# bcosm/MonteCarloOptionsPricer

Hardware: AMD Instinct MI355X
Metric: Mpaths/sec at 252 steps (higher is better)
Workload: dtype f64; 1 GPU; C2: European call, GBM, 10M paths x 252 steps per GPU, fp64 matrix written; collective=none, seed=20251031

## Files before the change

### include/mcgpu_debug.h

```cpp
#ifndef MCGPU_DEBUG_H
#define MCGPU_DEBUG_H
#include "mcgpu.h"
#ifdef __cplusplus
extern "C" {
#endif

int mcg_debug_eval(mcg_ctx* ctx, int fn, const double* x, double* y, int64_t n);
int mcg_debug_lsm_hooks(mcg_ctx* ctx, long long spin_limit, int poll_delay);
int mcg_debug_lsm_date_fault(mcg_ctx* ctx, int mode, int date, int workgroup, int delay, long long spin_limit);
int mcg_debug_batch_budget(mcg_ctx* ctx, size_t bytes);
int mcg_debug_coalesce_slots(int max_slots);
int mcg_debug_coalesce_selftest(int n_threads, int calls_per_thread, int* wrong);
int mcg_debug_peer_decision(int same_process, int bus_id_resolves, int same_device, int can_access_peer);
int mcg_debug_shm_attach(const char* name, int n_ranks, int rank, double timeout_s, void** handle);
int mcg_debug_shm_barrier(void* handle);
int mcg_debug_shm_poison(void* handle);
int mcg_debug_shm_detach(void* handle);

#ifdef __cplusplus
}
#endif
#endif
```

### montecarlooptionspricer_amd/_native.py

```python
from __future__ import annotations

import ctypes as C
import os
import sys

_HERE = os.path.dirname(os.path.abspath(__file__))
_LIB = os.environ.get("MCG_LIB") or os.path.join(_HERE, "lib", "libmcgpu.so")

MCG_OK = 0
K_GBM, K_RBERGOMI, K_PAYOFF, K_LSM_SWEEP, K_LSM_SOLVE, K_TRANSPOSE, K_ASYM, K_MARTINGALE, K_BRANCHING, K_BATCH, K_EXOTIC, K_HESTON, K_MULTI, K_LOCALVOL = range(14)
KERNEL_NAMES = {K_GBM: "gbm", K_RBERGOMI: "rbergomi", K_PAYOFF: "payoff", K_LSM_SWEEP: "lsm_sweep",
                K_LSM_SOLVE: "lsm_solve", K_TRANSPOSE: "transpose", K_ASYM: "asymptotic", K_MARTINGALE: "martingale", K_BRANCHING: "branching", K_BATCH: "batch_rows",
                K_EXOTIC: "exotic", K_HESTON: "heston", K_MULTI: "multi", K_LOCALVOL: "localvol"}
K_LSM_APPLY = 14

LSM_POLICY_STRIDE = 20
POL_CONTINUE, POL_EXERCISE_RULE, POL_TERMINAL = range(3)

(X_ASIAN_ARITH_FIXED, X_ASIAN_ARITH_FLOAT, X_ASIAN_GEO_FIXED, X_ASIAN_GEO_FLOAT, X_LOOKBACK_FIXED, X_LOOKBACK_FLOAT,
 X_BARRIER_UP_OUT, X_BARRIER_UP_IN, X_BARRIER_DOWN_OUT, X_BARRIER_DOWN_IN) = range(10)
EXOTIC_KINDS = {"asian_arith_fixed": X_ASIAN_ARITH_FIXED, "asian_arith_float": X_ASIAN_ARITH_FLOAT,
                "asian_geo_fixed": X_ASIAN_GEO_FIXED, "asian_geo_float": X_ASIAN_GEO_FLOAT,
                "lookback_fixed": X_LOOKBACK_FIXED, "lookback_float": X_LOOKBACK_FLOAT,
                "barrier_up_out": X_BARRIER_UP_OUT, "barrier_up_in": X_BARRIER_UP_IN,
# ... 100 lines not shown
                raise

    newer("mcg_comm_shm_peer_mailbox", [vp, C.c_int, C.POINTER(C.c_int)])
    newer("mcg_debug_shm_attach", [C.c_char_p, C.c_int, C.c_int, C.c_double, C.POINTER(vp)])
    newer("mcg_debug_shm_barrier", [vp])
    newer("mcg_debug_shm_poison", [vp])
    newer("mcg_debug_shm_detach", [vp])
    newer("mcg_lsm_one_launch_reset", [vp])
    newer("mcg_debug_lsm_hooks", [vp, C.c_longlong, C.c_int])
    newer("mcg_comm_info", [vp] + [C.POINTER(C.c_int)] * 4)
    newer("mcg_timing_select", [vp, C.c_uint])
    newer("mcg_stats", [C.POINTER(Stats), C.c_int])
    newer("mcg_debug_lsm_date_fault", [vp, C.c_int, C.c_int, C.c_int, C.c_int, C.c_longlong])
    newer("mcg_debug_batch_budget", [vp, C.c_size_t])
    newer("mcg_debug_peer_decision", [C.c_int] * 4)
    newer("mcg_probe_write_ceiling", [vp, C.c_int64, C.c_int, C.c_int, C.POINTER(C.c_double), C.POINTER(C.c_double)])
    newer("mcg_generator_clock_arm", [vp, C.c_int])
    newer("mcg_generator_clock", [vp, C.POINTER(C.c_double), C.POINTER(C.c_int), C.POINTER(C.c_double), C.POINTER(C.c_double)])
    newer("mcg_row_features", [C.POINTER(C.c_double), C.c_size_t, C.POINTER(C.c_double), C.POINTER(C.c_double)])
    newer("mcg_row_build", [C.POINTER(C.c_double), C.c_size_t, C.c_double, C.c_double, C.c_double, C.c_int, C.c_double,
                            C.POINTER(Row), C.POINTER(C.c_double)])
    newer("mcg_batch_price_rows6", [vp, C.POINTER(Row), C.POINTER(C.c_double), C.c_int64, C.c_int, C.c_double, C.c_double, C.c_int,
                                    C.c_int, C.c_int, C.c_uint64, C.POINTER(C.c_double)])
    L.mcg_paths_gbm.argtypes = [vp, C.c_uint64, C.c_double, C.c_double, C.c_double, C.c_double, C.c_int,
                                C.c_uint64, C.c_int64, C.POINTER(vp)]
    L.mcg_paths_gbm_payoff.argtypes = [vp, C.c_uint64, C.c_double, C.c_double, C.c_double, C.c_double, C.c_int,
                                       C.c_uint64, C.c_int64, C.c_double, C.c_int, C.POINTER(vp)]
    L.mcg_paths_rbergomi.argtypes = [vp, C.c_uint64] + [C.c_double] * 7 + [C.c_int, C.c_uint64, C.c_int64,
                                                                          C.POINTER(vp)]
    L.mcg_paths_rbergomi_payoff.argtypes = [vp, C.c_uint64] + [C.c_double] * 7 + [C.c_int, C.c_uint64, C.c_int64,
                                                                                 C.c_double, C.c_int, C.POINTER(vp)]
    L.mcg_paths_heston.argtypes = [vp, C.c_uint64] + [C.c_double] * 8 + [C.c_int, C.c_uint64, C.c_int64, C.POINTER(vp), C.POINTER(vp)]
    L.mcg_paths_heston_payoff.argtypes = [vp, C.c_uint64] + [C.c_double] * 8 + [C.c_int, C.c_uint64, C.c_int64, C.c_double, C.c_int,
                                          C.POINTER(vp), C.POINTER(vp)]
    L.mcg_paths_heston_qe.argtypes = L.mcg_paths_heston.argtypes
    L.mcg_paths_heston_qe_payoff.argtypes = L.mcg_paths_heston_payoff.argtypes
    L.mcg_paths_bates.argtypes = [vp, C.c_uint64] + [C.c_double] * 11 + [C.c_int, C.c_uint64, C.c_int64, C.c_int, C.POINTER(vp),
                                                                          C.POINTER(vp)]
    L.mcg_paths_bates_payoff.argtypes = [vp, C.c_uint64] + [C.c_double] * 11 + [C.c_int, C.c_uint64, C.c_int64, C.c_int, C.c_double,
                                                                                 C.c_int, C.POINTER(vp), C.POINTER(vp)]
    L.mcg_cholesky_corr.argtypes = [dp, C.c_int, dp]
    L.mcg_paths_gbm_multi.argtypes = [vp, C.c_uint64, C.c_int, dp, C.c_double, dp, dp, dp, C.c_double, C.c_int, C.c_uint64, C.c_int64,
                                      C.c_int, dp, C.POINTER(vp), C.POINTER(vp)]
    L.mcg_paths_combine.argtypes = [vp, C.POINTER(vp), C.c_int, C.c_int, dp, C.POINTER(vp)]
    lv = [vp, C.c_uint64, C.c_double, C.c_double, C.c_double, dp, C.c_int, C.c_double, C.c_double, C.c_int, dp, C.c_double, C.c_int,
          C.c_uint64, C.c_int64]
# ... 56 lines not shown
```

### montecarlooptionspricer_amd/csrc/fastmath.hpp

```cpp
#pragma once
#include <hip/hip_runtime.h>
#include <stdint.h>

#include "philox.hpp"

namespace mcg {
namespace fm {

constexpr int LOG_TAB_ENTRIES = 1024;
constexpr int SINCOS_BITS = 10;
constexpr int SINCOS_TAB_ENTRIES = 1 << SINCOS_BITS;
constexpr int EXP2_TAB_ENTRIES = 256;
constexpr int TABLE_UNITS = LOG_TAB_ENTRIES + SINCOS_TAB_ENTRIES + EXP2_TAB_ENTRIES / 2;

struct Tables {
    static constexpr int SC_BITS = SINCOS_BITS;
    double2 log[LOG_TAB_ENTRIES];
    double2 sincos[SINCOS_TAB_ENTRIES];
    double exp2[EXP2_TAB_ENTRIES];
};
template <int BITS>
struct NormalTables {
    static_assert(BITS >= 6 && BITS <= SINCOS_BITS, "a sub-sampling of the 1024-entry table");
    static constexpr int SC_BITS = BITS;
// ... 252 lines not shown
    z1 = rad * s;
}

template <class T>
__device__ __forceinline__ void box_muller_pair_affine(uint32_t wa, uint32_t wb, const T* tab, double scale,
                                                       double shift, double& a0, double& a1) {
    const double rad = scale * sqrt_pos(neg2log(radius_u01(wa, wb), tab->log));
    double c, s;
    sincos_table<T::SC_BITS>(wb, tab->sincos, c, s);
    a0 = __builtin_fma(rad, c, shift);
    a1 = __builtin_fma(rad, s, shift);
}

template <class T>
__device__ __forceinline__ void box_muller_pair_affine_scaled(uint32_t wa, uint32_t wb, const T* tab, const LogScale& L,
                                                              double shift, double& a0, double& a1) {
    const double rad = sqrt_pos(neg2log_scaled(radius_u01(wa, wb), tab->log, L));
    double c, s;
    sincos_table<T::SC_BITS>(wb, tab->sincos, c, s);
    a0 = __builtin_fma(rad, c, shift);
    a1 = __builtin_fma(rad, s, shift);
}

template <bool EAGER = false>
__device__ __forceinline__ void normal_quad_words(const Philox4 w, const Tables* tab, double (&z)[4], double amp0, double amp1);

template <bool EAGER = false>
__device__ __forceinline__ void normal_quad_fast(uint32_t k0, uint32_t k1, uint64_t path, uint32_t block,
                                                 uint32_t stream, const Tables* tab, double (&z)[4], double amp0 = 1.0,
                                                 double amp1 = 1.0) {
    normal_quad_words<EAGER>(philox4x32_10((uint32_t)path, (uint32_t)(path >> 32), block, stream, k0, k1), tab, z, amp0, amp1);
}
template <bool EAGER = false>
__device__ __forceinline__ void normal_quad_fast(uint32_t k0, uint32_t k1, const PhiloxLane& L, uint32_t block, const Tables* tab,
                                                 double (&z)[4], double amp0 = 1.0, double amp1 = 1.0) {
    normal_quad_words<EAGER>(philox4x32_10_path(L, block, k0, k1), tab, z, amp0, amp1);
}

template <bool EAGER>
__device__ __forceinline__ void normal_quad_words(const Philox4 w, const Tables* tab, double (&z)[4], double amp0, double amp1) {
    if constexpr (!EAGER) {
        box_muller_pair_affine(w.w0, w.w1, tab, amp0, 0.0, z[0], z[1]);
        box_muller_pair_affine(w.w2, w.w3, tab, amp1, 0.0, z[2], z[3]);
        return;
    }
    const LogSplit s0 = log_split(radius_u01(w.w0, w.w1)), s1 = log_split(radius_u01(w.w2, w.w3));
// ... 41 lines not shown
```

### montecarlooptionspricer_amd/csrc/kernels_debug.hip

```cpp
#include "devmath.hpp"
#include "fastmath.hpp"
#include "mcg_internal.hpp"

namespace mcg {

__global__ __launch_bounds__(256) void k_debug_eval(int fn, const double* x, double* y, int64_t n,
                                                    const double2* gtab) {
    __shared__ fm::Tables tabs;
    const fm::Tables* tab = &tabs;
    fm::load_tables(&tabs, gtab);
    __syncthreads();
    const int64_t i = (int64_t)blockIdx.x * 256 + threadIdx.x;
    if (i >= n) return;
    const double v = x[i];
    double a = 0.0, b = 0.0;
    double z[4] = {0.0, 0.0, 0.0, 0.0};
    switch (fn) {
        case 0: a = fm::scaled_exp(1.0, v); break;
        case 1: a = fm::neg2log(v, tab->log); break;
        case 2: a = fm::sqrt_pos(v); break;
        case 3: fm::sincos_table((uint32_t)v, tab->sincos, a, b); break;
        case 4: fm::normal_quad_fast(1u, 0u, (uint64_t)v, 0u, STREAM_PRICE, tab, z); break;
        case 6: a = fm::scaled_exp_small(1.0, v); break;
        case 7: a = fm::scaled_exp_small6(1.0, v); break;
        case 8: fm::exp2_pair(v, v + 96.0, tab, a, b); break;
        case 9: fm::normal_quad_fast<true>(1u, 0u, (uint64_t)v, 0u, STREAM_PRICE, tab, z); break;
        default: normal_quad_ref(1u, 0u, (uint64_t)v, 0u, STREAM_PRICE, z); break;
    }
    if (fn < 4 || (fn > 5 && fn != 9)) {
        z[0] = a;
        z[1] = b;
    }
#pragma unroll
    for (int e = 0; e < 4; ++e) y[4 * i + e] = z[e];
}

}

extern "C" int mcg_debug_eval(mcg_ctx* ctx, int fn, const double* x, double* y, int64_t n) {
    using namespace mcg;
    if (!ctx || !x || !y || n < 0 || fn < 0 || fn > 9) return fail(MCG_ERR_INVALID, "bad arguments");
    if (n == 0) return MCG_OK;
    MCG_HIP(hipSetDevice(ctx->device));
    double *dx = nullptr, *dy = nullptr;
    MCG_HIP(hipMalloc((void**)&dx, (size_t)n * sizeof(double)));
    if (hipMalloc((void**)&dy, (size_t)n * 4 * sizeof(double)) != hipSuccess) {
        (void)hipFree(dx);
        return fail(MCG_ERR_OOM, "hipMalloc failed");
    }
    int rc = MCG_OK;
    if (hipMemcpyAsync(dx, x, (size_t)n * sizeof(double), hipMemcpyHostToDevice, ctx->stream) != hipSuccess)
        rc = fail(MCG_ERR_HIP, "H2D failed");
    if (rc == MCG_OK) {
        hipLaunchKernelGGL(k_debug_eval, dim3((unsigned)((n + 255) / 256)), dim3(256), 0, ctx->stream, fn, dx, dy, n,
                           (const double2*)ctx->log_tab);
        if (hipMemcpyAsync(y, dy, (size_t)n * 4 * sizeof(double), hipMemcpyDeviceToHost, ctx->stream) != hipSuccess ||
            hipStreamSynchronize(ctx->stream) != hipSuccess)
            rc = fail(MCG_ERR_HIP, "debug eval failed: %s", hipGetErrorString(hipGetLastError()));
    }
    (void)hipFree(dx);
    (void)hipFree(dy);
    return rc;
}
```

### montecarlooptionspricer_amd/csrc/kernels_gbm.hip

```cpp
#include <algorithm>
#include <cstdlib>
#include <vector>

#include "devmath.hpp"
#include "fastmath.hpp"
#include "mcg_internal.hpp"

#ifndef MCG_GBM_TABLES
#define MCG_GBM_TABLES 0
#endif

namespace mcg {

struct GbmArgs {
    double* out;
    int64_t ld;
    int64_t n_paths;
    int n_steps;
    uint64_t path_begin;
    uint32_t k0, k1;
    double S0, drift, vol;
    fm::LogScale ls;
    double K;
    int is_call;
    double* partials;
    const double2* log_tab;
    unsigned long long* clk;
    unsigned clk_first, clk_shift;
};

template <bool PAYOFF, int MODE, int PPL>
__global__ __launch_bounds__(256) void k_gbm_paths(GbmArgs a) {
    constexpr bool SMALL = MODE >= 1;
    typedef double v2d __attribute__((ext_vector_type(2)));
#if MCG_GBM_TABLES == 0
    typedef fm::Tables GbmTables;
    __shared__ GbmTables tabs;
    if (MODE >= 2) fm::load_tables_scaled(&tabs, a.log_tab, a.vol * a.vol);
    else fm::load_tables(&tabs, a.log_tab);
#else
    typedef fm::NormalTables<MCG_GBM_TABLES == 1 ? 10 : 9> GbmTables;
    __shared__ GbmTables tabs;
    fm::load_normal_tables(&tabs, a.log_tab, MODE >= 2 ? a.vol * a.vol : 1.0);
#endif
    const GbmTables* tab = &tabs;
    __syncthreads();
#ifdef MCG_GBM_NO_STAMPS
    const bool stamps = false;
#else
    const bool stamps = a.clk != nullptr && (blockIdx.x & ((1u << a.clk_shift) - 1u)) == a.clk_first;
#endif
// ... 73 lines not shown
    if (threadIdx.x == 0 && stamp0[2] != 0) {
        const unsigned long long c1 = __builtin_amdgcn_s_memtime(), r1 = __builtin_amdgcn_s_memrealtime();
        unsigned long long* dst = (unsigned long long*)stamp0[2];
        dst[0] = c1 - stamp0[0];
        dst[1] = r1 - stamp0[1];
    }
    if (PAYOFF) {
        __shared__ double red[2 * 4];
        double v[2] = {0.0, 0.0};
#pragma unroll
        for (int p = 0; p < PPL; ++p) {
            const double pay = (in_row && i + p < a.n_paths) ? payoff_of(a.is_call != 0, S[p], a.K) : 0.0;
            v[0] += pay;
            v[1] += pay * pay;
        }
        block_sum<2, 4>(v, red);
        if (threadIdx.x == 0) {
            a.partials[2 * (int64_t)blockIdx.x] = v[0];
            a.partials[2 * (int64_t)blockIdx.x + 1] = v[1];
        }
    }
}

__global__ __launch_bounds__(256) void k_payoff_sums(const double* last_row, int64_t n_paths, double K,
                                                     int is_call, double* partials) {
    __shared__ double red[2 * 4];
    double v[2] = {0.0, 0.0};
    for (int64_t i = (int64_t)blockIdx.x * 256 + threadIdx.x; i < n_paths; i += (int64_t)gridDim.x * 256) {
        const double pay = payoff_of(is_call != 0, last_row[i], K);
        v[0] += pay;
        v[1] += pay * pay;
    }
    block_sum<2, 4>(v, red);
    if (threadIdx.x == 0) {
        partials[2 * (int64_t)blockIdx.x] = v[0];
        partials[2 * (int64_t)blockIdx.x + 1] = v[1];
    }
}

constexpr int64_t FIN_CHUNK = 8192;

__device__ __forceinline__ void sum_pairs(const double* partials, int64_t n, double (&v)[2], double* red) {
    v[0] = 0.0;
    v[1] = 0.0;
    for (int64_t b = threadIdx.x; b < n; b += 1024) {
        v[0] += partials[2 * b];
// ... 44 lines not shown
    }
    MCG_HIP(hipGetLastError());
    if (ctx->allreduce) {
        if (ctx->allreduce(ctx->allreduce_user, d, 3, (void*)ctx->stream) != 0)
            return fail(MCG_ERR_COMM, "all-reduce of payoff sums failed");
    }
    MCG_HIP(hipMemcpyAsync(ctx->h_scalars + SC_SUMS, d, 3 * sizeof(double), hipMemcpyDeviceToHost, ctx->stream));
    MCG_HIP(hipStreamSynchronize(ctx->stream));
    out3[0] = ctx->h_scalars[SC_SUMS];
    out3[1] = ctx->h_scalars[SC_SUMS + 1];
    out3[2] = ctx->h_scalars[SC_SUMS + 2];
    return MCG_OK;
}

template <bool PAYOFF, int PPL>
static void launch_gbm_mode(mcg_ctx* ctx, const GbmArgs& a, int mode, unsigned n_blocks) {
    const dim3 grid(n_blocks), block(256);
    if (mode == 3) hipLaunchKernelGGL((k_gbm_paths<PAYOFF, 3, PPL>), grid, block, 0, ctx->stream, a);
    else if (mode == 2) hipLaunchKernelGGL((k_gbm_paths<PAYOFF, 2, PPL>), grid, block, 0, ctx->stream, a);
    else if (mode == 1) hipLaunchKernelGGL((k_gbm_paths<PAYOFF, 1, PPL>), grid, block, 0, ctx->stream, a);
    else hipLaunchKernelGGL((k_gbm_paths<PAYOFF, 0, PPL>), grid, block, 0, ctx->stream, a);
}

static int gbm_paths_per_lane(const mcg_ctx* ctx, int64_t n_paths) {
    static const int forced = study_switch("MCG_GBM_PPL", 0);
    if (forced == 1 || forced == 2) return forced;
    return n_paths >= (int64_t)ctx->n_cus * 512 * 8 ? 2 : 1;
}

int launch_gbm(mcg_ctx* ctx, mcg_paths* P, uint64_t seed, double S0, double r, double sigma, double dt,
               bool want_payoff, double K, int is_call) {
    const int ppl = gbm_paths_per_lane(ctx, P->n_paths);
    const int64_t n_blocks = (P->n_paths + 256 * ppl - 1) / (256 * ppl);
    if (n_blocks > 0x7fffffffLL) return fail(MCG_ERR_INVALID, "n_paths too large for one launch");
    if ((P->ld & 255) != 0) return fail(MCG_ERR_INVALID, "path matrix rows must be padded to 256 columns");
    if (want_payoff) {
        int rc = ensure_cap(ctx, &ctx->partials, &ctx->partials_cap, (size_t)(2 * n_blocks));
        if (rc) return rc;
    }
    GbmArgs a;
    a.out = P->data;
    a.ld = P->ld;
    a.n_paths = P->n_paths;
    a.n_steps = P->n_steps;
    a.path_begin = P->path_begin;
    a.k0 = (uint32_t)seed;
    a.k1 = (uint32_t)(seed >> 32);
    a.S0 = S0;
    a.drift = (r - 0.5 * sigma * sigma) * dt;
    a.vol = sigma * std::sqrt(dt);
    a.K = K;
    a.is_call = is_call;
    a.partials = ctx->partials;
    a.log_tab = (const double2*)ctx->log_tab;
    a.clk = nullptr;
    a.clk_first = 0;
    a.clk_shift = 0;
    ctx->clk_slots_used = 0;
    if (ctx->clk_armed && ctx->clk_stamps && n_blocks >= 64) {
        unsigned shift = 2;
        while (((n_blocks - 1) >> shift) >= GBM_CLK_SLOTS) ++shift;
        a.clk = ctx->clk_stamps;
        a.clk_shift = shift;
        a.clk_first = (1u << shift) / 2;
        ctx->clk_slots_used = (int)(((n_blocks - 1 - a.clk_first) >> shift) + 1);
        MCG_HIP(hipMemsetAsync(ctx->clk_stamps, 0, sizeof(unsigned long long) * 2 * GBM_CLK_SLOTS, ctx->stream));
    }
    {
        TimedLaunch t(ctx, MCG_K_GBM);
        const bool small = std::fabs(a.drift) + std::fabs(a.vol) * fm::MAX_ABS_NORMAL <= fm::SMALL_EXP_BOUND;
        const double reach = std::fabs(a.drift) + std::fabs(a.vol) * fm::MAX_ABS_NORMAL;
        const int mode = !small ? 0 : !(a.vol > 1e-100) ? 1 : reach <= fm::SMALL6_EXP_BOUND ? 3 : 2;
        a.ls = fm::make_log_scale(a.vol * a.vol);
        if (want_payoff) {
            if (ppl == 2) launch_gbm_mode<true, 2>(ctx, a, mode, (unsigned)n_blocks);
            else launch_gbm_mode<true, 1>(ctx, a, mode, (unsigned)n_blocks);
        } else {
            if (ppl == 2) launch_gbm_mode<false, 2>(ctx, a, mode, (unsigned)n_blocks);
            else launch_gbm_mode<false, 1>(ctx, a, mode, (unsigned)n_blocks);
        }
    }
    MCG_HIP(hipGetLastError());
    if (want_payoff) return keep_sums(finish_sums(ctx, n_blocks, P->n_paths, P->sums), P, K, is_call);
    return MCG_OK;
}

int generator_clock(mcg_ctx* ctx, double* ghz_median, int* n_stamps, double* ghz_min, double* ghz_max) {
    if (ghz_median) *ghz_median = 0.0;
    if (n_stamps) *n_stamps = 0;
    if (ghz_min) *ghz_min = 0.0;
    if (ghz_max) *ghz_max = 0.0;
    if (!ctx->clk_stamps || ctx->clk_slots_used < 1) return MCG_OK;
    unsigned long long h[2 * GBM_CLK_SLOTS];
    MCG_HIP(hipStreamSynchronize(ctx->stream));
    MCG_HIP(hipMemcpy(h, ctx->clk_stamps, sizeof h, hipMemcpyDeviceToHost));
    std::vector<double> g;
    for (int k = 0; k < ctx->clk_slots_used; ++k)
// ... 26 lines not shown
```

### montecarlooptionspricer_amd/csrc/mcg_api.hip

```cpp
#include <algorithm>
#include <cmath>
#include <cstdlib>
#include <cstring>
#include <new>
#include <vector>

#include "fastmath_tables.hpp"
#include "mcg_internal.hpp"

namespace mcg {

static thread_local std::string g_err;
Stats g_stats;

void set_error(const char* fmt, ...) {
    char buf[512];
    va_list ap;
    va_start(ap, fmt);
    vsnprintf(buf, sizeof buf, fmt, ap);
    va_end(ap);
    g_err = buf;
}

int fail(int status, const char* fmt, ...) {
// ... 205 lines not shown
        ctx->owns_stream = false;
    } else {
        hipError_t se = hipStreamCreateWithFlags(&ctx->stream, hipStreamNonBlocking);
        if (se != hipSuccess) {
            delete ctx;
            return fail(MCG_ERR_HIP, "hipStreamCreate failed: %s", hipGetErrorString(se));
        }
        ctx->owns_stream = true;
    }
    if (hipMalloc((void**)&ctx->scalars, SCALARS_DOUBLES * sizeof(double)) != hipSuccess ||
        hipMalloc((void**)&ctx->clk_stamps, sizeof(unsigned long long) * 2 * GBM_CLK_SLOTS) != hipSuccess ||
        hipHostMalloc((void**)&ctx->h_scalars, SCALARS_DOUBLES * sizeof(double)) != hipSuccess) {
        mcg_finalize(ctx);
        return fail(MCG_ERR_OOM, "workspace allocation failed");
    }
    constexpr size_t n_log = sizeof(fm::LOG_TAB_HOST) / sizeof(double), n_sc = sizeof(fm::SINCOS_TAB_HOST) / sizeof(double);
    if (hipMalloc((void**)&ctx->log_tab, sizeof(fm::LOG_TAB_HOST) + sizeof(fm::SINCOS_TAB_HOST) + sizeof(fm::EXP2_TAB_HOST)) != hipSuccess ||
        hipMemcpy(ctx->log_tab, fm::LOG_TAB_HOST, sizeof(fm::LOG_TAB_HOST), hipMemcpyHostToDevice) != hipSuccess ||
        hipMemcpy(ctx->log_tab + n_log, fm::SINCOS_TAB_HOST, sizeof(fm::SINCOS_TAB_HOST), hipMemcpyHostToDevice) != hipSuccess ||
        hipMemcpy(ctx->log_tab + n_log + n_sc, fm::EXP2_TAB_HOST, sizeof(fm::EXP2_TAB_HOST), hipMemcpyHostToDevice) != hipSuccess) {
        mcg_finalize(ctx);
        return fail(MCG_ERR_OOM, "table upload failed");
    }
    *out = ctx;
    return MCG_OK;
}

int mcg_init(mcg_ctx** out, int device) { return init_impl(out, device, false, nullptr); }

int mcg_init_on_stream(mcg_ctx** out, int device, void* stream) { return init_impl(out, device, true, stream); }

int mcg_finalize(mcg_ctx* ctx) {
    if (!ctx) return MCG_OK;
    (void)hipSetDevice(ctx->device);
    if (ctx->stream) (void)hipStreamSynchronize(ctx->stream);
    comm_release(ctx);
    shm_release(ctx);
    for (mcg_paths* P : ctx->live_paths) {
        if (P->data) (void)hipFree(P->data);
        P->data = nullptr;
        P->ctx = nullptr;
    }
    ctx->live_paths.clear();
    for (auto& b : ctx->pool) (void)hipFree(b.ptr);
    ctx->pool.clear();
    for (auto& kv : ctx->ev_live) {
        (void)hipEventDestroy(kv.second.a);
        (void)hipEventDestroy(kv.second.b);
    }
    for (auto& ev : ctx->ev_free) {
        (void)hipEventDestroy(ev.a);
        (void)hipEventDestroy(ev.b);
    }
    if (ctx->partials) (void)hipFree(ctx->partials);
    if (ctx->fin_chunks) (void)hipFree(ctx->fin_chunks);
    if (ctx->scalars) (void)hipFree(ctx->scalars);
    if (ctx->clk_stamps) (void)hipFree(ctx->clk_stamps);
    if (ctx->h_scalars) (void)hipHostFree(ctx->h_scalars);
    if (ctx->weights) (void)hipFree(ctx->weights);
    if (ctx->lsm_v) (void)hipFree(ctx->lsm_v);
    if (ctx->lsm_dv) (void)hipFree(ctx->lsm_dv);
    if (ctx->log_tab) (void)hipFree(ctx->log_tab);
    if (ctx->batch_fork) (void)hipEventDestroy(ctx->batch_fork);
    if (ctx->batch_join) (void)hipEventDestroy(ctx->batch_join);
    if (ctx->batch_aux) (void)hipStreamDestroy(ctx->batch_aux);
    if (ctx->owns_stream && ctx->stream) (void)hipStreamDestroy(ctx->stream);
    delete ctx;
    return MCG_OK;
}

int mcg_synchronize(mcg_ctx* ctx) {
    if (!ctx) return fail(MCG_ERR_INVALID, "ctx is NULL");
    MCG_HIP(hipStreamSynchronize(ctx->stream));
    return MCG_OK;
}

int mcg_trim(mcg_ctx* ctx) {
    if (!ctx) return fail(MCG_ERR_INVALID, "ctx is NULL");
    MCG_HIP(hipStreamSynchronize(ctx->stream));
    for (auto& b : ctx->pool) (void)hipFree(b.ptr);
    ctx->pool.clear();
    return MCG_OK;
}

int mcg_set_allreduce(mcg_ctx* ctx, mcg_allreduce_fn fn, void* user) {
// ... 772 lines not shown
                                   &g_stats.coalesced_rounds, &g_stats.coalesced_calls, &g_stats.coalesced_peak_calls_per_round,
                                   &g_stats.coalesced_fallbacks, &g_stats.coalesced_round_us, &g_stats.coalesced_device_wait_us,
                                   &g_stats.coalesced_wake_us, &g_stats.coalesced_prefetched, &g_stats.coalesced_prefetch_hits};
    static_assert(sizeof(mcg_stats_t) == sizeof(src) / sizeof(src[0]) * sizeof(int64_t), "mcg_stats_t lists the counters in this order");
    int64_t* dst = reinterpret_cast<int64_t*>(out);
    for (size_t k = 0; k < sizeof(src) / sizeof(src[0]); ++k) {
        const int64_t v = reset ? src[k]->exchange(0, std::memory_order_relaxed) : src[k]->load(std::memory_order_relaxed);
        if (out) dst[k] = v;
    }
    return MCG_OK;
}

int mcg_debug_lsm_date_fault(mcg_ctx* ctx, int mode, int date, int workgroup, int delay, long long spin_limit) {
    if (!ctx) return fail(MCG_ERR_INVALID, "ctx is NULL");
    if (mode < 0 || mode > 2 || delay < 0 || delay > 100000 || spin_limit > 0xffffffffLL) return fail(MCG_ERR_INVALID, "bad hook values");
    ctx->lsm_date_hook[0] = mode;
    ctx->lsm_date_hook[1] = date;
    ctx->lsm_date_hook[2] = workgroup;
    ctx->lsm_date_hook[3] = delay;
    ctx->lsm_date_spin_limit = spin_limit;
    return MCG_OK;
}

int mcg_debug_batch_budget(mcg_ctx* ctx, size_t bytes) {
    if (!ctx) return fail(MCG_ERR_INVALID, "ctx is NULL");
    ctx->batch_budget = bytes;
    return MCG_OK;
}

int mcg_estimate_params(const double* hist, size_t n, double out5[5]) {
    if (!out5) return fail(MCG_ERR_INVALID, "out5 is NULL");
    return host_estimate_params(hist, n, out5);
}

int mcg_rbergomi_spectrum(double H, double eta, double dt, int n_steps, double* amp, double* comp, int* Mz) {
    if (n_steps < 1 || !amp || !comp) return fail(MCG_ERR_INVALID, "bad arguments");
    std::vector<double> k, c;
    int rc = host_rbergomi_spectrum(H, eta, dt, n_steps, k, c);
    if (rc) return rc;
    std::memcpy(amp, k.data(), k.size() * sizeof(double));
    std::memcpy(comp, c.data(), c.size() * sizeof(double));
    if (Mz) *Mz = (int)k.size();
    return MCG_OK;
}

int mcg_timing_enable(mcg_ctx* ctx, int on) {
// ... 32 lines not shown
```

### montecarlooptionspricer_amd/csrc/mcg_internal.hpp

```cpp
#pragma once
#include <hip/hip_runtime.h>
#include <stdint.h>

#include <algorithm>
#include <atomic>
#include <cmath>
#include <cstdarg>
#include <cstdio>
#include <cstdlib>
#include <string>
#include <utility>
#include <vector>

#include "../../include/mcgpu.h"
#include "../../include/mcgpu_debug.h"

namespace mcg {

void set_error(const char* fmt, ...);
int fail(int status, const char* fmt, ...);

inline int study_switch(const char* name, int fallback) {
#ifdef MCG_STUDY_SWITCHES
    if (const char* e = std::getenv(name)) return std::atoi(e);
// ... 52 lines not shown
    int lsm_date_hook[4] = {0, 0, 0, 0};
    size_t batch_budget = 0;
    hipStream_t batch_aux = nullptr;
    hipEvent_t batch_fork = nullptr, batch_join = nullptr;

    std::vector<mcg::PoolBuf> pool;
    std::vector<mcg_paths*> live_paths;
    double* partials = nullptr;
    size_t partials_cap = 0;
    double* fin_chunks = nullptr;
    size_t fin_chunks_cap = 0;
    double* scalars = nullptr;
    double* h_scalars = nullptr;
    double* weights = nullptr;
    size_t weights_cap = 0;
    double* lsm_v = nullptr;
    size_t lsm_v_cap = 0;
    double* lsm_dv = nullptr;
    size_t lsm_dv_cap = 0;
    unsigned long long* clk_stamps = nullptr;
    int clk_slots_used = 0;
    bool clk_armed = false;
    double* log_tab = nullptr;

    mcg_allreduce_fn allreduce = nullptr;
    void* allreduce_user = nullptr;
    void* rccl_comm = nullptr;
    mcg::ShmComm* shm = nullptr;
    int n_ranks = 1, rank = 0;

    bool timing = false;
    unsigned timing_mask = ~0u;
    std::vector<mcg::EventPair> ev_free;
    std::vector<std::pair<int, mcg::EventPair>> ev_live;
    double t_total[MCG_K_COUNT] = {0};
    int64_t t_count[MCG_K_COUNT] = {0};
};

struct mcg_paths {
    mcg_ctx* ctx = nullptr;
    double* data = nullptr;
    size_t bytes = 0;
    int64_t n_paths = 0;
    int n_steps = 0;
    int64_t ld = 0;
    uint64_t path_begin = 0;
    bool generated = false;
    bool has_sums = false;
    double sums_K = 0.0;
    int sums_is_call = 0;
    double sums[3] = {0, 0, 0};
};

namespace mcg {

constexpr int GBM_CLK_SLOTS = 64;
constexpr int SCALARS_DOUBLES = 256;
constexpr int SC_SUMS = 0;
constexpr int SC_GREEKS = 4;
constexpr int SC_COEF = 40;
constexpr int SC_FINAL = 64;
constexpr int SC_BARRIER = 72;
constexpr int SC_TICKET = 80;
constexpr int SC_LSM_TICKET = 160;
constexpr int SC_LSM_MSG = 96;
constexpr int SC_LSM_STATE = 144;

int pool_alloc(mcg_ctx* ctx, size_t bytes, void** out);
void pool_release(mcg_ctx* ctx, void* ptr, size_t bytes);
int ensure_cap(mcg_ctx* ctx, double** buf, size_t* cap, size_t need_doubles);

struct TimedLaunch {
    mcg_ctx* ctx;
    int kernel;
    EventPair ev{};
    bool on;
    TimedLaunch(mcg_ctx* c, int k, int64_t launches = 1);
    ~TimedLaunch();
};

void comm_release(mcg_ctx* ctx);
int comm_rccl_count(mcg_ctx* ctx);
void shm_release(mcg_ctx* ctx);
int shm_arm_mailbox(mcg_ctx* ctx, int rounds, uint64_t sentinel_bits);
int shm_sum_flag(mcg_ctx* ctx, int flag, int* total);
void shm_poison(mcg_ctx* ctx);
// ... 66 lines not shown
int run_lsm_greeks(mcg_ctx* ctx, const mcg_paths* P, double r, double K, double maturity, double dt, int is_call,
                   int poly_order, mcg_greeks* out);
int greeks_lsm_final(mcg_ctx* ctx, const mcg_paths* P, double K, const double* V, const double* dV, mcg_greeks* out);
int run_path_stats(mcg_ctx* ctx, const mcg_paths* P, int first_row, double* host_out5);
int run_exotics(mcg_ctx* ctx, const mcg_paths* P, double r, double T, int first_row, const mcg_exotic* book, int n_contracts,
                double* price, double* std_err, double* sums);
int launch_path_stats(mcg_ctx* ctx, const mcg_paths* P, int first_row, bool geo, double* d_stats);
int exotic_allreduce_sums(mcg_ctx* ctx, double* d, int count);
int exotic_args(mcg_ctx* ctx, const mcg_paths* P, int first_row);
int exotic_contract_check(const mcg_exotic& x, const char* what, int index);

int lsm_reduce_allreduce_solve(mcg_ctx* ctx, int grid, int nm, int nb, double min_count, double K, int mo_mode, double mo_mu);
int run_martingale(mcg_ctx* ctx, const mcg_paths* P, double r, double K, double maturity, double dt, int is_call,
                   int poly_order, int max_iterations, double* price, double* lower, double* upper);
int run_branching(mcg_ctx* ctx, const mcg_paths* P, double r, double K, double maturity, double dt, int is_call,
                  int num_branches, const int* exercise_times, int n_ex, uint64_t seed, double* price, double* lower,
                  double* upper);
int run_batch_rows(mcg_ctx* ctx, const mcg_row* rows, int64_t n_rows, int n_paths, double r, double dt, int num_branches,
                   int poly_order, int max_iterations, uint64_t seed, double* out, unsigned char* priced);
int probe_write_ceiling(mcg_ctx* ctx, int64_t n_paths, int n_steps, int reps, double* gb_per_s, double* ms_per_launch);
int run_asymptotic(mcg_ctx* ctx, const mcg_paths* P, double r, double K, double maturity, double dt, int is_call,
                   double sigma, double dividend, double* price);

void host_asymptotic_tables(int n_cols, double r, double K, double maturity, double dt, int is_call, double sigma,
                            double dividend, std::vector<double>& bnd, std::vector<double>& disc);
int host_estimate_params(const double* hist, size_t n, double out5[5]);
void host_row_features(const double* hist, size_t n, double* vol, double* momentum);
int host_row_build(const double* hist, size_t n, double underlying_last, double dte, double strike_dist_pct, int option_type,
                   double dividend, mcg_row* row, double features2[2]);
int host_rbergomi_spectrum(double H, double eta, double dt, int n_steps, std::vector<double>& amp,
                           std::vector<double>& comp);
int localvol_check_surface(const double* times, int n_t, int n_x, const double* sigma, double dt, int n_steps);
int localvol_check_model(double S0, double r, double q, double x_min, double x_max, bool payoff, double K);
void localvol_fill_table(const double* times, int n_t, int n_x, const double* sigma, double dt, int n_steps, double* table);
LocalVolScalars localvol_scalars(double r, double q, double x_min, double x_max, int n_x, double dt);

}
```

### montecarlooptionspricer_amd/engine.py

```python
from __future__ import annotations

import ctypes as C
import math
import weakref
from typing import Callable, Optional, Tuple

import numpy as np

from . import _native as N
from ._native import McgError, check


class _DevView:

    def __init__(self, ptr: int, count: int):
        self.__cuda_array_interface__ = {"shape": (count,), "typestr": "<f8", "data": (ptr, False),
                                         "version": 3, "strides": None}


class PathMatrix:

    def __init__(self, engine: "PathEngine", handle: C.c_void_p):
        self._engine = engine
        self._h = handle
# ... 427 lines not shown
    def debug_lsm_date_fault(self, mode: int = 0, date: int = 0, workgroup: int = 0, delay: int = 0, spin_limit: int = -1) -> None:
        check(self._L.mcg_debug_lsm_date_fault(self._ctx, int(mode), int(date), int(workgroup), int(delay), int(spin_limit)))

    def probe_write_ceiling(self, n_paths: int = 10_000_000, n_steps: int = 252, reps: int = 5) -> Tuple[float, float]:
        g, ms = C.c_double(), C.c_double()
        check(self._L.mcg_probe_write_ceiling(self._ctx, int(n_paths), int(n_steps), int(reps), C.byref(g), C.byref(ms)))
        return g.value, ms.value

    def generator_clock_arm(self, on: bool = True) -> None:
        check(self._L.mcg_generator_clock_arm(self._ctx, 1 if on else 0))

    def generator_clock(self) -> dict:
        med, lo, hi, n = C.c_double(), C.c_double(), C.c_double(), C.c_int()
        check(self._L.mcg_generator_clock(self._ctx, C.byref(med), C.byref(n), C.byref(lo), C.byref(hi)))
        return {"GHz_median": med.value, "GHz_min": lo.value, "GHz_max": hi.value, "stamping_workgroups": n.value}

    def debug_eval(self, fn: int, x: np.ndarray) -> np.ndarray:
        x = np.ascontiguousarray(x, dtype=np.float64)
        y = np.empty((len(x), 4), dtype=np.float64)
        check(self._L.mcg_debug_eval(self._ctx, int(fn), x.ctypes.data_as(C.POINTER(C.c_double)),
                                     y.ctypes.data_as(C.POINTER(C.c_double)), len(x)))
        return y

    def timing_enable(self, on: bool = True) -> None:
        check(self._L.mcg_timing_enable(self._ctx, int(on)))

    def timing_select(self, kernels=None) -> None:
        mask = 0xFFFFFFFF if kernels is None else sum(1 << int(k) for k in kernels)
        check(self._L.mcg_timing_select(self._ctx, mask))

    def timing_reset(self) -> None:
        check(self._L.mcg_timing_reset(self._ctx))

    def timing_get(self, kernel: int) -> Tuple[float, int]:
        ms, n = C.c_double(), C.c_int64()
        check(self._L.mcg_timing_get(self._ctx, kernel, C.byref(ms), C.byref(n)))
        return ms.value, n.value


def _vec(x) -> np.ndarray:
    return np.ascontiguousarray(np.atleast_1d(np.asarray(x, dtype=np.float64)))


def _combine_kind(kind) -> int:
    if isinstance(kind, str):
        if kind.lower() not in N.COMBINE_KINDS:
# ... 237 lines not shown
    s = N.Stats()
    check(L.mcg_stats(C.byref(s), int(bool(reset))))
    return {k: int(getattr(s, k)) for k, _ in N.Stats._fields_}


def estimate_params(hist) -> dict:
    L = N.load_library()
    h = np.ascontiguousarray(hist, dtype=np.float64)
    out = np.empty(5)
    check(L.mcg_estimate_params(h.ctypes.data_as(C.POINTER(C.c_double)), len(h), out.ctypes.data_as(C.POINTER(C.c_double))))
    return dict(xi=out[0], H=out[1], eta=out[2], rho=out[3], S0=out[4])


def rbergomi_spectrum(H: float, eta: float, dt: float, n_steps: int):
    L = N.load_library()
    M = 1
    while M < n_steps:
        M *= 2
    amp, comp, mz = np.empty(M), np.empty(n_steps), C.c_int()
    check(L.mcg_rbergomi_spectrum(H, eta, dt, n_steps, amp.ctypes.data_as(C.POINTER(C.c_double)),
                                  comp.ctypes.data_as(C.POINTER(C.c_double)), C.byref(mz)))
    assert mz.value == M
    return amp, comp
```

Baseline: 2405 Mpaths/s.

## Add wide persistent GBM kernel with two-level sincos tables and tile tickets

```diff
diff --git a/include/mcgpu_debug.h b/include/mcgpu_debug.h
--- a/include/mcgpu_debug.h
+++ b/include/mcgpu_debug.h
@@ -6,6 +6,8 @@
 #endif
 
 int mcg_debug_eval(mcg_ctx* ctx, int fn, const double* x, double* y, int64_t n);
+int mcg_debug_sincos2_tables(double* coarse, double* fine);
+int mcg_debug_gbm_route(mcg_ctx* ctx, int route, int* last_route);
 int mcg_debug_lsm_hooks(mcg_ctx* ctx, long long spin_limit, int poll_delay);
 int mcg_debug_lsm_date_fault(mcg_ctx* ctx, int mode, int date, int workgroup, int delay, long long spin_limit);
 int mcg_debug_batch_budget(mcg_ctx* ctx, size_t bytes);
diff --git a/montecarlooptionspricer_amd/_native.py b/montecarlooptionspricer_amd/_native.py
--- a/montecarlooptionspricer_amd/_native.py
+++ b/montecarlooptionspricer_amd/_native.py
@@ -146,6 +146,8 @@
                             C.POINTER(Row), C.POINTER(C.c_double)])
     newer("mcg_batch_price_rows6", [vp, C.POINTER(Row), C.POINTER(C.c_double), C.c_int64, C.c_int, C.c_double, C.c_double, C.c_int,
                                     C.c_int, C.c_int, C.c_uint64, C.POINTER(C.c_double)])
+    newer("mcg_debug_sincos2_tables", [dp, dp])
+    newer("mcg_debug_gbm_route", [vp, C.c_int, C.POINTER(C.c_int)])
     L.mcg_paths_gbm.argtypes = [vp, C.c_uint64, C.c_double, C.c_double, C.c_double, C.c_double, C.c_int,
                                 C.c_uint64, C.c_int64, C.POINTER(vp)]
     L.mcg_paths_gbm_payoff.argtypes = [vp, C.c_uint64, C.c_double, C.c_double, C.c_double, C.c_double, C.c_int,
diff --git a/montecarlooptionspricer_amd/csrc/fastmath.hpp b/montecarlooptionspricer_amd/csrc/fastmath.hpp
--- a/montecarlooptionspricer_amd/csrc/fastmath.hpp
+++ b/montecarlooptionspricer_amd/csrc/fastmath.hpp
@@ -298,6 +298,50 @@
     a1 = __builtin_fma(rad, s, shift);
 }
 
+constexpr int SINCOS2_BITS = 12;
+constexpr int SINCOS2_ENTRIES = 1 << SINCOS2_BITS;
+__device__ __forceinline__ void sincos_two_level_entries(const double2 C, const double2 F, double& c_out, double& s_out) {
+    c_out = __builtin_fma(C.x, F.x, -(C.y * F.y));
+    s_out = __builtin_fma(C.y, F.x, C.x * F.y);
+}
+__device__ __forceinline__ void sincos_two_level(uint32_t wb, const double2* coarse, const double2* fine, double& c_out,
+                                                 double& s_out) {
+    sincos_two_level_entries(coarse[wb >> (32 - SINCOS2_BITS)], fine[(wb >> 8) & (SINCOS2_ENTRIES - 1u)], c_out, s_out);
+}
+
+__device__ __forceinline__ double neg2log_entry_scaled(const LogSplit& sp, const double2 e, const LogScale& L) {
+    const double r = __builtin_fma(sp.z, e.x, -1.0);
+    double q = L.q3;
+    q = fma_sc(q, r, L.q2);
+    q = fma_sc(q, r, L.q1);
+    q = fma_sc(q, r, L.q0);
+    const double P = __builtin_fma(r, q, L.c_l);
+    const double base = __builtin_fma((double)sp.k, L.c_k, e.y);
+    return __builtin_fma(r, P, base);
+}
+
+__device__ __forceinline__ void box_muller_pair_affine2(uint32_t wa, uint32_t wb, const double2* log_tab, const double2* coarse,
+                                                        const double2* fine, double scale, double shift, double& a0, double& a1) {
+    const LogSplit sp = log_split(radius_u01(wa, wb));
+    const double2 L = log_tab[sp.idx], C = coarse[wb >> (32 - SINCOS2_BITS)], F = fine[(wb >> 8) & (SINCOS2_ENTRIES - 1u)];
+    const double rad = scale * sqrt_pos(neg2log_entry(sp, L));
+    double c, s;
+    sincos_two_level_entries(C, F, c, s);
+    a0 = __builtin_fma(rad, c, shift);
+    a1 = __builtin_fma(rad, s, shift);
+}
+__device__ __forceinline__ void box_muller_pair_affine_scaled2(uint32_t wa, uint32_t wb, const double2* log_tab,
+                                                               const double2* coarse, const double2* fine, const LogScale& Ls,
+                                                               double shift, double& a0, double& a1) {
+    const LogSplit sp = log_split(radius_u01(wa, wb));
+    const double2 L = log_tab[sp.idx], C = coarse[wb >> (32 - SINCOS2_BITS)], F = fine[(wb >> 8) & (SINCOS2_ENTRIES - 1u)];
+    const double rad = sqrt_pos(neg2log_entry_scaled(sp, L, Ls));
+    double c, s;
+    sincos_two_level_entries(C, F, c, s);
+    a0 = __builtin_fma(rad, c, shift);
+    a1 = __builtin_fma(rad, s, shift);
+}
+
 template <bool EAGER = false>
 __device__ __forceinline__ void normal_quad_words(const Philox4 w, const Tables* tab, double (&z)[4], double amp0, double amp1);
 
diff --git a/montecarlooptionspricer_amd/csrc/kernels_debug.hip b/montecarlooptionspricer_amd/csrc/kernels_debug.hip
--- a/montecarlooptionspricer_amd/csrc/kernels_debug.hip
+++ b/montecarlooptionspricer_amd/csrc/kernels_debug.hip
@@ -5,7 +5,7 @@
 namespace mcg {
 
 __global__ __launch_bounds__(256) void k_debug_eval(int fn, const double* x, double* y, int64_t n,
-                                                    const double2* gtab) {
+                                                    const double2* gtab, const double2* sincos2) {
     __shared__ fm::Tables tabs;
     const fm::Tables* tab = &tabs;
     fm::load_tables(&tabs, gtab);
@@ -25,6 +25,7 @@
         case 7: a = fm::scaled_exp_small6(1.0, v); break;
         case 8: fm::exp2_pair(v, v + 96.0, tab, a, b); break;
         case 9: fm::normal_quad_fast<true>(1u, 0u, (uint64_t)v, 0u, STREAM_PRICE, tab, z); break;
+        case 10: fm::sincos_two_level((uint32_t)v, sincos2, sincos2 + fm::SINCOS2_ENTRIES, a, b); break;
         default: normal_quad_ref(1u, 0u, (uint64_t)v, 0u, STREAM_PRICE, z); break;
     }
     if (fn < 4 || (fn > 5 && fn != 9)) {
@@ -39,7 +40,7 @@
 
 extern "C" int mcg_debug_eval(mcg_ctx* ctx, int fn, const double* x, double* y, int64_t n) {
     using namespace mcg;
-    if (!ctx || !x || !y || n < 0 || fn < 0 || fn > 9) return fail(MCG_ERR_INVALID, "bad arguments");
+    if (!ctx || !x || !y || n < 0 || fn < 0 || fn > 10) return fail(MCG_ERR_INVALID, "bad arguments");
     if (n == 0) return MCG_OK;
     MCG_HIP(hipSetDevice(ctx->device));
     double *dx = nullptr, *dy = nullptr;
@@ -53,7 +54,7 @@
         rc = fail(MCG_ERR_HIP, "H2D failed");
     if (rc == MCG_OK) {
         hipLaunchKernelGGL(k_debug_eval, dim3((unsigned)((n + 255) / 256)), dim3(256), 0, ctx->stream, fn, dx, dy, n,
-                           (const double2*)ctx->log_tab);
+                           (const double2*)ctx->log_tab, (const double2*)ctx->sincos2_tab);
         if (hipMemcpyAsync(y, dy, (size_t)n * 4 * sizeof(double), hipMemcpyDeviceToHost, ctx->stream) != hipSuccess ||
             hipStreamSynchronize(ctx->stream) != hipSuccess)
             rc = fail(MCG_ERR_HIP, "debug eval failed: %s", hipGetErrorString(hipGetLastError()));
diff --git a/montecarlooptionspricer_amd/csrc/kernels_gbm.hip b/montecarlooptionspricer_amd/csrc/kernels_gbm.hip
--- a/montecarlooptionspricer_amd/csrc/kernels_gbm.hip
+++ b/montecarlooptionspricer_amd/csrc/kernels_gbm.hip
@@ -27,6 +27,9 @@
     const double2* log_tab;
     unsigned long long* clk;
     unsigned clk_first, clk_shift;
+    const double2* sincos2;
+    unsigned* ticket;
+    unsigned n_tiles;
 };
 
 template <bool PAYOFF, int MODE, int PPL>
@@ -146,6 +149,132 @@
     }
 }
 
+struct WideTables {
+    double2 log[fm::LOG_TAB_ENTRIES];
+    double2 coarse[fm::SINCOS2_ENTRIES];
+    double2 fine[fm::SINCOS2_ENTRIES];
+};
+constexpr int WIDE_WAVES = 16, WIDE_TILE = 128;
+static_assert(fm::SINCOS2_ENTRIES == SINCOS2_ENTRIES, "host/sincos2.cpp builds what fm::sincos_two_level indexes");
+static_assert(sizeof(WideTables) == 147456, "144 KiB: one workgroup per CU");
+
+template <bool PAYOFF, int MODE>
+__global__ __launch_bounds__(64 * WIDE_WAVES) void k_gbm_paths_wide(GbmArgs a) {
+    constexpr bool SMALL = MODE >= 1;
+    typedef double v2d __attribute__((ext_vector_type(2)));
+    __shared__ WideTables tabs;
+    __shared__ unsigned long long stamp0[WIDE_WAVES][2];
+    {
+        const double scale = a.vol * a.vol;
+        for (int i = threadIdx.x; i < fm::LOG_TAB_ENTRIES; i += 64 * WIDE_WAVES) {
+            double2 e = a.log_tab[i];
+            if (MODE >= 2) e.y *= scale;
+            tabs.log[i] = e;
+        }
+        double2* sc = reinterpret_cast<double2*>(&tabs) + fm::LOG_TAB_ENTRIES;
+        for (int i = threadIdx.x; i < 2 * fm::SINCOS2_ENTRIES; i += 64 * WIDE_WAVES) sc[i] = a.sincos2[i];
+    }
+    __syncthreads();
+    const unsigned lane = threadIdx.x & 63u;
+    const unsigned wave = __builtin_amdgcn_readfirstlane(threadIdx.x >> 6);
+    const unsigned lane_bytes = lane * 16u;
+    typedef const __attribute__((address_space(4))) GbmArgs* TileArgs;
+    auto tile_args = [] {
+        TileArgs p = (TileArgs)__builtin_amdgcn_kernarg_segment_ptr();
+        asm volatile("" : "+s"(p));
+        return p;
+    };
+    auto stamping = [](TileArgs t, unsigned tile) {
+        return t->clk != nullptr && (tile & ((1u << t->clk_shift) - 1u)) == t->clk_first && (tile >> t->clk_shift) < (unsigned)GBM_CLK_SLOTS;
+    };
+    unsigned tile = blockIdx.x * WIDE_WAVES + wave;
+    while (tile < tile_args()->n_tiles) {
+        const TileArgs t = tile_args();
+        if (stamping(t, tile) && lane == 0) {
+            stamp0[wave][0] = __builtin_amdgcn_s_memtime();
+            stamp0[wave][1] = __builtin_amdgcn_s_memrealtime();
+        }
+        const int64_t col = (int64_t)tile * WIDE_TILE + lane * 2;
+        double S[2] = {t->S0, t->S0};
+        double* row = t->out + (int64_t)tile * WIDE_TILE;
+        auto store_row = [&](double* r) {
+            const v2d v = {S[0], S[1]};
+            asm volatile("global_store_dwordx4 %0, %1, %2 nt\n\ts_nop 1" : : "v"(lane_bytes), "v"(v), "s"(r) : "memory");
+        };
+        store_row(row);
+        PhiloxLane lane_rng[2];
+#pragma unroll
+        for (int p = 0; p < 2; ++p) lane_rng[p] = philox_lane_setup(t->path_begin + (uint64_t)(col + p), STREAM_PRICE, a.k1);
+        auto step = [&](const double (&e)[2]) {
+#pragma unroll
+            for (int p = 0; p < 2; ++p)
+                S[p] = MODE == 3 ? fm::scaled_exp_small6(S[p], e[p]) : SMALL ? fm::scaled_exp_small(S[p], e[p]) : fm::scaled_exp(S[p], e[p]);
+            row += a.ld;
+            store_row(row);
+        };
+        auto pair_exponents = [&](uint32_t wa, uint32_t wb, double& e0, double& e1) {
+            if (MODE >= 2) fm::box_muller_pair_affine_scaled2(wa, wb, tabs.log, tabs.coarse, tabs.fine, a.ls, a.drift, e0, e1);
+            else fm::box_muller_pair_affine2(wa, wb, tabs.log, tabs.coarse, tabs.fine, a.vol, a.drift, e0, e1);
+        };
+        const int n_blocks = a.n_steps >> 2;
+#pragma unroll 1
+        for (int b = 0; b < n_blocks; ++b) {
+            Philox4 w[2];
+#pragma unroll
+            for (int p = 0; p < 2; ++p) w[p] = philox4x32_10_lane(lane_rng[p], (uint32_t)b, a.k0, a.k1);
+            double e0[2], e1[2];
+#pragma unroll
+            for (int p = 0; p < 2; ++p) pair_exponents(w[p].w0, w[p].w1, e0[p], e1[p]);
+            step(e0);
+            step(e1);
+#pragma unroll
+            for (int p = 0; p < 2; ++p) pair_exponents(w[p].w2, w[p].w3, e0[p], e1[p]);
+            step(e0);
+            step(e1);
+        }
+        const int rest = tile_args()->n_steps & 3;
+        if (rest) {
+            Philox4 w[2];
+#pragma unroll
+            for (int p = 0; p < 2; ++p) w[p] = philox4x32_10_lane(lane_rng[p], (uint32_t)n_blocks, a.k0, a.k1);
+            double e0[2], e1[2];
+#pragma unroll
+            for (int p = 0; p < 2; ++p) pair_exponents(w[p].w0, w[p].w1, e0[p], e1[p]);
+            step(e0);
+            if (rest >= 2) step(e1);
+            if (rest == 3) {
+#pragma unroll
+                for (int p = 0; p < 2; ++p) pair_exponents(w[p].w2, w[p].w3, e0[p], e1[p]);
+                step(e0);
+            }
+        }
+        const TileArgs e = tile_args();
+        if (stamping(e, tile) && lane == 0) {
+            const unsigned long long c1 = __builtin_amdgcn_s_memtime(), r1 = __builtin_amdgcn_s_memrealtime();
+            unsigned long long* dst = e->clk + 2 * (tile >> e->clk_shift);
+            dst[0] = c1 - stamp0[wave][0];
+            dst[1] = r1 - stamp0[wave][1];
+        }
+        if (PAYOFF) {
+            double v[2] = {0.0, 0.0};
+#pragma unroll
+            for (int p = 0; p < 2; ++p) {
+                const double pay = col + p < e->n_paths ? payoff_of(e->is_call != 0, S[p], e->K) : 0.0;
+                v[0] += pay;
+                v[1] += pay * pay;
+            }
+            wave_sum_all<2>(v);
+            if (lane == 0) {
+                e->partials[2 * (int64_t)tile] = v[0];
+                e->partials[2 * (int64_t)tile + 1] = v[1];
+            }
+        }
+        unsigned drawn = 0;
+        if (lane == 0) drawn = atomicAdd(e->ticket, 1u);
+        tile = __builtin_amdgcn_readfirstlane(drawn) + gridDim.x * WIDE_WAVES;
+    }
+}
+
 __global__ __launch_bounds__(256) void k_payoff_sums(const double* last_row, int64_t n_paths, double K,
                                                      int is_call, double* partials) {
     __shared__ double red[2 * 4];
@@ -236,6 +365,22 @@
     else hipLaunchKernelGGL((k_gbm_paths<PAYOFF, 0, PPL>), grid, block, 0, ctx->stream, a);
 }
 
+template <bool PAYOFF>
+static void launch_gbm_wide_mode(mcg_ctx* ctx, const GbmArgs& a, int mode) {
+    const unsigned n_groups = std::min<unsigned>((unsigned)ctx->n_cus, (a.n_tiles + WIDE_WAVES - 1) / WIDE_WAVES);
+    const dim3 grid(n_groups), block(64 * WIDE_WAVES);
+    if (mode == 3) hipLaunchKernelGGL((k_gbm_paths_wide<PAYOFF, 3>), grid, block, 0, ctx->stream, a);
+    else if (mode == 2) hipLaunchKernelGGL((k_gbm_paths_wide<PAYOFF, 2>), grid, block, 0, ctx->stream, a);
+    else if (mode == 1) hipLaunchKernelGGL((k_gbm_paths_wide<PAYOFF, 1>), grid, block, 0, ctx->stream, a);
+    else hipLaunchKernelGGL((k_gbm_paths_wide<PAYOFF, 0>), grid, block, 0, ctx->stream, a);
+}
+
+constexpr int64_t GBM_WIDE_MIN_PATHS = 2000000;
+static bool gbm_takes_wide(const mcg_ctx* ctx, int64_t n_paths) {
+    if (ctx->gbm_route == 1 || ctx->gbm_route == 2) return ctx->gbm_route == 2;
+    return n_paths >= GBM_WIDE_MIN_PATHS;
+}
+
 static int gbm_paths_per_lane(const mcg_ctx* ctx, int64_t n_paths) {
     static const int forced = study_switch("MCG_GBM_PPL", 0);
     if (forced == 1 || forced == 2) return forced;
@@ -244,10 +389,11 @@
 
 int launch_gbm(mcg_ctx* ctx, mcg_paths* P, uint64_t seed, double S0, double r, double sigma, double dt,
                bool want_payoff, double K, int is_call) {
+    const bool wide = gbm_takes_wide(ctx, P->n_paths);
     const int ppl = gbm_paths_per_lane(ctx, P->n_paths);
-    const int64_t n_blocks = (P->n_paths + 256 * ppl - 1) / (256 * ppl);
+    if ((P->ld & 255) != 0) return fail(MCG_ERR_INVALID, "path matrix rows must be padded to 256 columns");
+    const int64_t n_blocks = wide ? P->ld / WIDE_TILE : (P->n_paths + 256 * ppl - 1) / (256 * ppl);
     if (n_blocks > 0x7fffffffLL) return fail(MCG_ERR_INVALID, "n_paths too large for one launch");
-    if ((P->ld & 255) != 0) return fail(MCG_ERR_INVALID, "path matrix rows must be padded to 256 columns");
     if (want_payoff) {
         int rc = ensure_cap(ctx, &ctx->partials, &ctx->partials_cap, (size_t)(2 * n_blocks));
         if (rc) return rc;
@@ -267,6 +413,9 @@
     a.is_call = is_call;
     a.partials = ctx->partials;
     a.log_tab = (const double2*)ctx->log_tab;
+    a.sincos2 = (const double2*)ctx->sincos2_tab;
+    a.ticket = reinterpret_cast<unsigned*>(ctx->scalars + SC_GBM_TICKET);
+    a.n_tiles = wide ? (unsigned)n_blocks : 0u;
     a.clk = nullptr;
     a.clk_first = 0;
     a.clk_shift = 0;
@@ -280,13 +429,18 @@
         ctx->clk_slots_used = (int)(((n_blocks - 1 - a.clk_first) >> shift) + 1);
         MCG_HIP(hipMemsetAsync(ctx->clk_stamps, 0, sizeof(unsigned long long) * 2 * GBM_CLK_SLOTS, ctx->stream));
     }
+    if (wide) MCG_HIP(hipMemsetAsync(a.ticket, 0, sizeof(unsigned), ctx->stream));
+    ctx->gbm_last_route = wide ? 2 : 1;
     {
         TimedLaunch t(ctx, MCG_K_GBM);
         const bool small = std::fabs(a.drift) + std::fabs(a.vol) * fm::MAX_ABS_NORMAL <= fm::SMALL_EXP_BOUND;
         const double reach = std::fabs(a.drift) + std::fabs(a.vol) * fm::MAX_ABS_NORMAL;
         const int mode = !small ? 0 : !(a.vol > 1e-100) ? 1 : reach <= fm::SMALL6_EXP_BOUND ? 3 : 2;
         a.ls = fm::make_log_scale(a.vol * a.vol);
-        if (want_payoff) {
+        if (wide) {
+            if (want_payoff) launch_gbm_wide_mode<true>(ctx, a, mode);
+            else launch_gbm_wide_mode<false>(ctx, a, mode);
+        } else if (want_payoff) {
             if (ppl == 2) launch_gbm_mode<true, 2>(ctx, a, mode, (unsigned)n_blocks);
             else launch_gbm_mode<true, 1>(ctx, a, mode, (unsigned)n_blocks);
         } else {
diff --git a/montecarlooptionspricer_amd/csrc/mcg_api.hip b/montecarlooptionspricer_amd/csrc/mcg_api.hip
--- a/montecarlooptionspricer_amd/csrc/mcg_api.hip
+++ b/montecarlooptionspricer_amd/csrc/mcg_api.hip
@@ -251,6 +251,12 @@
         mcg_finalize(ctx);
         return fail(MCG_ERR_OOM, "table upload failed");
     }
+    constexpr size_t sincos2_bytes = sizeof(double) * 4 * SINCOS2_ENTRIES;
+    if (hipMalloc((void**)&ctx->sincos2_tab, sincos2_bytes) != hipSuccess ||
+        hipMemcpy(ctx->sincos2_tab, host_sincos2_tables(), sincos2_bytes, hipMemcpyHostToDevice) != hipSuccess) {
+        mcg_finalize(ctx);
+        return fail(MCG_ERR_OOM, "table upload failed");
+    }
     *out = ctx;
     return MCG_OK;
 }
@@ -290,6 +296,7 @@
     if (ctx->lsm_v) (void)hipFree(ctx->lsm_v);
     if (ctx->lsm_dv) (void)hipFree(ctx->lsm_dv);
     if (ctx->log_tab) (void)hipFree(ctx->log_tab);
+    if (ctx->sincos2_tab) (void)hipFree(ctx->sincos2_tab);
     if (ctx->batch_fork) (void)hipEventDestroy(ctx->batch_fork);
     if (ctx->batch_join) (void)hipEventDestroy(ctx->batch_join);
     if (ctx->batch_aux) (void)hipStreamDestroy(ctx->batch_aux);
@@ -1108,6 +1115,14 @@
     return MCG_OK;
 }
 
+int mcg_debug_gbm_route(mcg_ctx* ctx, int route, int* last_route) {
+    if (!ctx) return fail(MCG_ERR_INVALID, "ctx is NULL");
+    if (route < -1 || route > 2) return fail(MCG_ERR_INVALID, "route must be 0 (auto), 1 (narrow), 2 (wide) or -1 (unchanged)");
+    if (route >= 0) ctx->gbm_route = route;
+    if (last_route) *last_route = ctx->gbm_last_route;
+    return MCG_OK;
+}
+
 int mcg_debug_batch_budget(mcg_ctx* ctx, size_t bytes) {
     if (!ctx) return fail(MCG_ERR_INVALID, "ctx is NULL");
     ctx->batch_budget = bytes;
diff --git a/montecarlooptionspricer_amd/csrc/mcg_internal.hpp b/montecarlooptionspricer_amd/csrc/mcg_internal.hpp
--- a/montecarlooptionspricer_amd/csrc/mcg_internal.hpp
+++ b/montecarlooptionspricer_amd/csrc/mcg_internal.hpp
@@ -98,6 +98,9 @@
     int clk_slots_used = 0;
     bool clk_armed = false;
     double* log_tab = nullptr;
+    double* sincos2_tab = nullptr;
+    int gbm_route = 0;
+    int gbm_last_route = 0;
 
     mcg_allreduce_fn allreduce = nullptr;
     void* allreduce_user = nullptr;
@@ -130,6 +133,7 @@
 
 namespace mcg {
 
+constexpr int SINCOS2_ENTRIES = 4096;
 constexpr int GBM_CLK_SLOTS = 64;
 constexpr int SCALARS_DOUBLES = 256;
 constexpr int SC_SUMS = 0;
@@ -138,6 +142,7 @@
 constexpr int SC_FINAL = 64;
 constexpr int SC_BARRIER = 72;
 constexpr int SC_TICKET = 80;
+constexpr int SC_GBM_TICKET = 81;
 constexpr int SC_LSM_TICKET = 160;
 constexpr int SC_LSM_MSG = 96;
 constexpr int SC_LSM_STATE = 144;
@@ -250,6 +255,7 @@
 int run_asymptotic(mcg_ctx* ctx, const mcg_paths* P, double r, double K, double maturity, double dt, int is_call,
                    double sigma, double dividend, double* price);
 
+const double* host_sincos2_tables();
 void host_asymptotic_tables(int n_cols, double r, double K, double maturity, double dt, int is_call, double sigma,
                             double dividend, std::vector<double>& bnd, std::vector<double>& disc);
 int host_estimate_params(const double* hist, size_t n, double out5[5]);
diff --git a/montecarlooptionspricer_amd/engine.py b/montecarlooptionspricer_amd/engine.py
--- a/montecarlooptionspricer_amd/engine.py
+++ b/montecarlooptionspricer_amd/engine.py
@@ -473,6 +473,11 @@
                                      y.ctypes.data_as(C.POINTER(C.c_double)), len(x)))
         return y
 
+    def debug_gbm_route(self, route: int = -1) -> int:
+        last = C.c_int()
+        check(self._L.mcg_debug_gbm_route(self._ctx, int(route), C.byref(last)))
+        return last.value
+
     def timing_enable(self, on: bool = True) -> None:
         check(self._L.mcg_timing_enable(self._ctx, int(on)))
 
@@ -756,3 +761,10 @@
                                   comp.ctypes.data_as(C.POINTER(C.c_double)), C.byref(mz)))
     assert mz.value == M
     return amp, comp
+
+
+def sincos2_tables():
+    L = N.load_library()
+    coarse, fine = np.empty((4096, 2)), np.empty((4096, 2))
+    check(L.mcg_debug_sincos2_tables(coarse.ctypes.data_as(C.POINTER(C.c_double)), fine.ctypes.data_as(C.POINTER(C.c_double))))
+    return coarse, fine
diff --git a/montecarlooptionspricer_amd/host/sincos2.cpp b/montecarlooptionspricer_amd/host/sincos2.cpp
--- /dev/null
+++ b/montecarlooptionspricer_amd/host/sincos2.cpp
@@ -0,0 +1,64 @@
+#include <cmath>
+#include <mutex>
+
+#include "../csrc/mcg_internal.hpp"
+
+namespace mcg {
+
+namespace {
+
+constexpr long double TWO_PI_L = 6.283185307179586476925286766559005768L;
+
+void octant_entry(int i, double& c_out, double& s_out) {
+    const int oct = i >> 9, k = i & 511;
+    const bool flip = (oct & 1) != 0;
+    const int kk = flip ? 512 - k : k;
+    const long double t = TWO_PI_L * (long double)kk / 4096.0L;
+    long double c = cosl(t), s = sinl(t);
+    if (kk == 0) {
+        c = 1.0L;
+        s = 0.0L;
+    }
+    if (flip) std::swap(c, s);
+    switch (oct >> 1) {
+        case 0: break;
+        case 1: { const long double x = c; c = -s; s = x; break; }
+        case 2: c = -c; s = -s; break;
+        default: { const long double x = c; c = s; s = -x; break; }
+    }
+    c_out = (double)c + 0.0;
+    s_out = (double)s + 0.0;
+}
+
+struct Sincos2Host {
+    double coarse[2 * SINCOS2_ENTRIES], fine[2 * SINCOS2_ENTRIES];
+};
+
+}
+
+const double* host_sincos2_tables() {
+    static Sincos2Host* tabs = nullptr;
+    static std::once_flag once;
+    std::call_once(once, [] {
+        Sincos2Host* t = new Sincos2Host;
+        for (int i = 0; i < SINCOS2_ENTRIES; ++i) {
+            octant_entry(i, t->coarse[2 * i], t->coarse[2 * i + 1]);
+            const long double a = TWO_PI_L * ((long double)i + 0.5L) / 16777216.0L;
+            t->fine[2 * i] = (double)cosl(a);
+            t->fine[2 * i + 1] = (double)sinl(a);
+        }
+        tabs = t;
+    });
+    return tabs->coarse;
+}
+
+}
+
+extern "C" int mcg_debug_sincos2_tables(double* coarse, double* fine) {
+    using namespace mcg;
+    if (!coarse || !fine) return fail(MCG_ERR_INVALID, "coarse or fine is NULL");
+    const double* t = host_sincos2_tables();
+    std::copy(t, t + 2 * SINCOS2_ENTRIES, coarse);
+    std::copy(t + 2 * SINCOS2_ENTRIES, t + 4 * SINCOS2_ENTRIES, fine);
+    return MCG_OK;
+}
```

Result: faster. 2636 Mpaths/s, median of 6 (+9.6%).
